# UDC-GAC/pRIblast

Measured on AMD Instinct MI355X. Metric: query RNAs/sec in `ris` step, higher is better.
Workload: dtype f64

## Files before the change

### priblast_amd/csrc/gapped_front.hip

```cpp
#include <algorithm>
#include <cstdlib>

#include "gapped_args.hpp"
#include "search_device.hpp"
#include "search_kernels.hpp"

namespace prb {

#ifdef PRB_GAP_PROFILE
__device__ unsigned long long g_front_prof[32];
#define FP_DECL unsigned long long fp_t0_ = __builtin_amdgcn_s_memtime(), fp_acc_[32] = {}
#define FP_MARK(k)                                              \
  do {                                                          \
    const unsigned long long t_ = __builtin_amdgcn_s_memtime(); \
    fp_acc_[k] += t_ - fp_t0_;                                  \
    fp_t0_ = t_;                                                \
  } while (0)
#define FP_COUNT(k, v) fp_acc_[k] += (unsigned long long)(v)
#define FP_FLUSH()                                                        \
  do {                                                                    \
    if (lane == 0)                                                        \
      for (int i_ = 0; i_ < 32; i_++) atomicAdd(&g_front_prof[i_], fp_acc_[i_]); \
  } while (0)
#else
#define FP_DECL
#define FP_MARK(k)
#define FP_COUNT(k, v)
#define FP_FLUSH()
#endif

namespace {

constexpr int kFD = kFrontMaxDrop;
#ifndef PRB_FRONT_RING
#define PRB_FRONT_RING 24
#endif
constexpr int kFR = PRB_FRONT_RING;
constexpr int kFWaves = 1;
constexpr int kFDirs = 64;
constexpr int kFCells = 192;
#ifndef PRB_FRONT_PAIRS
#define PRB_FRONT_PAIRS 256
#endif
constexpr int kFPairs = PRB_FRONT_PAIRS;

struct FrontTab {
  static constexpr int kBulge = SearchTab::kInt11;
  static constexpr int kTau = kBulge + 31;
  static constexpr int kZero = kTau + 8;
  static constexpr int kCount = kZero + 1;
};
static_assert(SearchTab::kStack == 0 && SearchTab::kInt11 == 255, "stack, internal and mismatch tables lead SearchTab");

struct FrontAcc {
  double eq[kFD][kFDirs], ed[kFD][kFDirs];
};

#ifndef PRB_FRONT_POOL
#define PRB_FRONT_POOL 832
#endif
constexpr int kFPool = PRB_FRONT_POOL;
static_assert(kFPool >= 2 * kFDirs && kFPool <= 1024, "FRec::pool");
static_assert(kFrontMaxDrop <= 16, "FrontLds::wfp: 16 cells per anti-diagonal");
struct FRec {
  static __device__ __forceinline__ uint32_t pack(int i, int j, int pool, int type, int qa, int da) {
    return (uint32_t)i | ((uint32_t)j << 5) | ((uint32_t)pool << 10) | ((uint32_t)type << 20) | ((uint32_t)qa << 23) | ((uint32_t)da << 26);
  }
  static __device__ __forceinline__ int i(uint32_t v) { return v & 31; }
  static __device__ __forceinline__ int j(uint32_t v) { return (v >> 5) & 31; }
  static __device__ __forceinline__ int pool(uint32_t v) { return (v >> 10) & 1023; }
  static __device__ __forceinline__ int type(uint32_t v) { return (v >> 20) & 7; }
  static __device__ __forceinline__ int qa(uint32_t v) { return (v >> 23) & 7; }
  static __device__ __forceinline__ int da(uint32_t v) { return (v >> 26) & 7; }
};

struct FrontLds {
  double hyb[kFPool];
  double te[kFPairs];
  int32_t tab[FrontTab::kCount];
  uint32_t info[kFR][kFDirs];
  uint32_t cells[kFCells];
  uint32_t wfp[2][kFDirs];
  uint8_t improved[kFDirs];
  uint32_t pairs[kFPairs];
};

struct Planes {
  uint32_t lo, hi, valid;
};
__device__ __forceinline__ int plane_base(uint32_t lo, uint32_t hi, uint32_t valid, int t) {
  const uint32_t l = (lo >> t) & 1, h = (hi >> t) & 1, v = (valid >> t) & 1;
  return v ? (int)(((h * 2 + l + 2) & 3) + 1) : 0;
}

__device__ __forceinline__ Planes load_planes(const uint8_t *s, int64_t n, int64_t start, int dir) {
  Planes p{0, 0, 0};
  const int64_t first = dir > 0 ? start : start - 31;
  const uintptr_t addr = reinterpret_cast<uintptr_t>(s) + (uintptr_t)first;
  const int sh = (int)(addr & 3);
  const uint32_t *sw = reinterpret_cast<const uint32_t *>(addr - (uintptr_t)sh);
  uint32_t w[9];
#pragma unroll
  for (int k = 0; k < 9; k++) {
    const int64_t pos_lo = first - sh + 4 * k;
    w[k] = (pos_lo + 3 >= 0 && pos_lo < n) ? sw[k] : 0u;
  }
  uint32_t x[8];
#pragma unroll
  for (int k = 0; k < 8; k++) x[k] = __builtin_amdgcn_alignbyte(w[k + 1], w[k], (uint32_t)sh);
#pragma unroll
  for (int k = 0; k < 8; k++) {
    const uint32_t c = x[k];
    const uint32_t any = (c | (c >> 1) | (c >> 2)) >> 1;
    const uint32_t lo4 = ((c & 0x01010101u) * 0x10204080u) >> 28;
    const uint32_t hi4 = (((c >> 1) & 0x01010101u) * 0x10204080u) >> 28;
    const uint32_t ok4 = ((any & 0x01010101u) * 0x10204080u) >> 28;
    p.lo |= lo4 << (4 * k);
    p.hi |= hi4 << (4 * k);
    p.valid |= ok4 << (4 * k);
  }
  {
    const int64_t lo_t = first < 0 ? -first : 0;
    const int64_t hi_t = first + 31 >= n ? n - 1 - first : 31;
    uint32_t inside = 0;
    if (hi_t >= lo_t) inside = (hi_t >= 31 ? ~0u : ((1u << (hi_t + 1)) - 1u)) & ~((1u << lo_t) - 1u);
    p.valid &= inside;
  }
  if (dir < 0) {
    p.lo = __builtin_bitreverse32(p.lo);
    p.hi = __builtin_bitreverse32(p.hi);
    p.valid = __builtin_bitreverse32(p.valid);
  }
  p.lo &= p.valid;
  p.hi &= p.valid;
  return p;
}

__device__ __forceinline__ void diag_masks(const Planes &q, const Planes &dr, int len, uint32_t &pairs, uint32_t &wob) {
  const int s = 31 - len;
  const uint32_t dl = dr.lo >> s, dh = dr.hi >> s, dv = dr.valid >> s;
  const uint32_t both = q.valid & dv, ldiff = q.lo ^ dl;
  const uint32_t gu = ~(q.hi | dh);
  wob = both & ldiff & gu;
  pairs = both & ldiff & ((q.hi ^ dh) | gu);
}

__device__ __forceinline__ int wave_excl_scan(int v, int lane, int &total) {
  int x = v;
  x += __builtin_amdgcn_update_dpp(0, x, 0x111, 0xF, 0xF, true);
  x += __builtin_amdgcn_update_dpp(0, x, 0x112, 0xF, 0xF, true);
  x += __builtin_amdgcn_update_dpp(0, x, 0x114, 0xF, 0xF, true);
  x += __builtin_amdgcn_update_dpp(0, x, 0x118, 0xF, 0xF, true);
  x += __builtin_amdgcn_update_dpp(0, x, 0x142, 0xA, 0xF, false);
  x += __builtin_amdgcn_update_dpp(0, x, 0x143, 0xC, 0xF, false);
  (void)lane;
  total = __builtin_amdgcn_readlane(x, 63);
  return x - v;
}

__device__ __forceinline__ void wave_lds_sync() {
  __builtin_amdgcn_fence(__ATOMIC_RELEASE, "wavefront");
  __builtin_amdgcn_wave_barrier();
  __builtin_amdgcn_fence(__ATOMIC_ACQUIRE, "wavefront");
}
__device__ __forceinline__ void wave_mem_sync() {
  __builtin_amdgcn_fence(__ATOMIC_RELEASE, "workgroup");
  __builtin_amdgcn_wave_barrier();
  __builtin_amdgcn_fence(__ATOMIC_ACQUIRE, "workgroup");
}

__device__ __forceinline__ double loop_energy_front(const SearchConst &sc, const int32_t *lt, int type, int type2, int u1, int u2, int a,
                                                    int b, int c, int d) {
  using T = SearchTab;
  using F = FrontTab;
  const int tt = type * 8 + type2;
  const int st = T::kStack + type * 7 + type2;
  const bool z1 = u1 == 0, z2 = u2 == 0;
  const int u = z1 ? u2 : u1;
  const bool c11 = u1 == 1 && u2 == 1, c12 = u1 == 1 && u2 == 2, c21 = u1 == 2 && u2 == 1, c22 = u1 == 2 && u2 == 2;
  const bool special = c11 || c12 || c21 || c22;
  int i1 = T::kInternal + u1 + u2;
  int i2 = special ? F::kZero : T::kMismatchI + (type * 5 + a) * 5 + b;
  int i3 = special ? F::kZero : T::kMismatchI + (type2 * 5 + d) * 5 + c;
  if (z1 || z2) {
    const bool stack = z1 && z2;
    i1 = stack ? st : F::kBulge + u;
    i2 = stack ? F::kZero : (u == 1 ? st : F::kTau + type);
    i3 = (stack || u == 1) ? F::kZero : F::kTau + type2;
  }
  int z1v = lt[special ? F::kZero : i1];
  if (special) {
    const int i11 = T::kInt11 + (tt * 5 + a) * 5 + b;
    const int i21a = T::kInt21 + ((tt * 5 + a) * 5 + d) * 5 + b;
    const int i21b = T::kInt21 + (((type2 * 8 + type) * 5 + d) * 5 + a) * 5 + c;
    const int i22 = T::kInt22 + (((tt * 5 + a) * 5 + c) * 5 + d) * 5 + b;
    z1v = sc.tab[c11 ? i11 : c12 ? i21a : c21 ? i21b : i22];
  }
  return div100(sc, z1v + lt[i2] + lt[i3]);
}

template <bool kOneDir>
__global__ __launch_bounds__(64 * kFWaves) void k_gapped_front(GapArgs a, FrontAcc *acc_blocks) {
  __shared__ FrontLds lds[kFWaves];
  const int lane = threadIdx.x & 63;
  FrontLds &S = lds[threadIdx.x >> 6];
  FrontAcc &A = acc_blocks[(int64_t)blockIdx.x * kFWaves + (threadIdx.x >> 6)];
  const SearchConst &sc = a.sc;
  for (int t = lane; t < FrontTab::kCount; t += 64)
    S.tab[t] = t < SearchTab::kInt11    ? sc.tab[t]
               : t < FrontTab::kTau     ? sc.tab[SearchTab::kBulge + (t - FrontTab::kBulge)]
               : t < FrontTab::kZero    ? sc.tab[SearchTab::kTau + (t - FrontTab::kTau)]
                                        : 0;
  const int flag = kOneDir ? 1 : lane & 1;
  const bool f0 = flag == 0;
  const int drop = a.o.drop_w_gap, min_helix = a.o.min_helix, delta = a.o.delta;
  const int64_t nwaves = (int64_t)gridDim.x * kFWaves;
  constexpr int kTileHits = kOneDir ? kFDirs : kFDirs / 2;
  const int64_t ntiles = (a.n + kTileHits - 1) / kTileHits;
  const bool isdir = lane < kFDirs;
  const int me = isdir ? lane : 0;
  int64_t tile = (int64_t)blockIdx.x * kFWaves + (threadIdx.x >> 6);
  FP_DECL;
  while (tile < ntiles) {
    FP_MARK(0);
    FP_COUNT(16, 1);
    unsigned long long nt = 0;
    if (lane == 0) nt = atomicAdd(a.next_work, 1ull);
    const int64_t w = tile * kTileHits + (kOneDir ? lane : lane >> 1);
    const bool live = isdir && w < a.n;
    int64_t x = 0, qo = 0, dbase = 0;
    int query = 0, id = 0, qn = 1, q_sp = 0, db_sp = 0, q_len = 0, db_len = 0, id_start = 0;
    double e_tot = 0, e_acc = 0;
    bool resumed = false;
    int tier0 = 0, nleft0 = 0;
    if (live) {
      x = a.subset ? (int64_t)a.subset[w] : w;
      query = a.in.query[x];
      qo = a.qb.off[query];
      qn = a.qb.len[query] + 1;
      id = a.in.db_id[x];
      dbase = (int64_t)a.pg.start_pos[id] - id;
      q_sp = a.in.q_sp[x];
      db_sp = a.in.db_sp[x];
      q_len = a.in.q_len[x];
      db_len = a.in.db_len[x];
      id_start = a.in.db_id_start[x];
      e_tot = a.in.e_tot[x];
      e_acc = a.in.e_acc[x];
      const uint8_t mark = a.tier_out[x];
      if (is_resumed(mark)) {
        resumed = true;
        tier0 = mark & kMarkTier;
        nleft0 = a.bp_count[x] & 0xFFFF;
        q_sp = a.out.q_sp[x];
        db_sp = a.out.db_sp[x];
        q_len = a.out.q_len[x];
        db_len = a.out.db_len[x];
        id_start = a.out.db_id_start[x];
        e_tot = a.out.e_tot[x];
        e_acc = a.out.e_acc[x];
      }
    }
    const uint8_t *qs = a.qb.enc + qo;
    const int q_start = f0 ? q_sp : q_sp + US(q_len) - 1;
    const int64_t db_start = f0 ? (int64_t)db_sp : (int64_t)db_sp + US(db_len) - 1;
    const int id_end = id_start + US(db_len) - 1;
    bool dead = !live || (resumed && f0);
    if (kOneDir && !resumed) dead = true;
    FP_MARK(1);

    Planes q{0, 0, 0}, dr{0, 0, 0};
    int tq0 = 1, td0 = 1;
    int type0 = 0, q1 = 0, d1 = 0;
    if (live) {
      q = load_planes(qs, qn, q_start, f0 ? -1 : 1);
      const Planes dd = load_planes(a.pg.seqs, a.pg.nchars, db_start, f0 ? -1 : 1);
      tq0 = (q.valid >> 1) == 0x7FFFFFFFu ? 32 : __builtin_ctz(~(q.valid >> 1)) + 1;
      td0 = (dd.valid >> 1) == 0x7FFFFFFFu ? 32 : __builtin_ctz(~(dd.valid >> 1)) + 1;
      const int q0 = plane_base(q.lo, q.hi, q.valid, 0), d0 = plane_base(dd.lo, dd.hi, dd.valid, 0);
      q1 = plane_base(q.lo, q.hi, q.valid, 1);
      d1 = plane_base(dd.lo, dd.hi, dd.valid, 1);
      type0 = bp_type(sc, q0, d0);
      if (f0) type0 = rtype_of(type0);
      dr.lo = __builtin_bitreverse32(dd.lo);
      dr.hi = __builtin_bitreverse32(dd.hi);
      dr.valid = __builtin_bitreverse32(dd.valid);
    }
    FP_MARK(2);
    const int open_until = tq0 > td0 ? tq0 : td0;
    const int lend = drop < open_until ? drop : open_until;

    {
      const float *a3 = f0 ? a.qb.acc + qo : a.pg.acc + dbase, *c3 = f0 ? a.qb.cond + qo : a.pg.cond + dbase;
      const float *c1 = f0 ? a.pg.cond + dbase + id_end : a.qb.cond + qo + q_start;
      const int p0 = f0 ? q_start : id_start;
      const int t3 = f0 ? tq0 : td0, t1 = f0 ? td0 : tq0;
      double s3 = 0, s1 = 0;
      float ta[kFD + 1], tz[kFD], tw[kFD];
      ta[0] = (live && 1 < t3 && 1 <= lend) ? a3[p0] : 0.0f;
#pragma unroll
      for (int len = 1; len <= kFD; len++) {
        const bool v3 = live && len < t3 && len <= lend, v1 = live && len < t1 && len <= lend;
        ta[len] = v3 ? a3[p0 - len] : 0.0f;
        tz[len - 1] = v3 ? c3[p0 - len + delta] : 0.0f;
        tw[len - 1] = v1 ? c1[len] : 0.0f;
      }
#pragma unroll
      for (int len = 1; len <= kFD; len++) {
        const float xx = ta[len], yy = ta[len - 1], zz = tz[len - 1], ww = tw[len - 1];
        s3 = len == 1 ? (double)(xx - yy + zz) : s3 + xx - yy + zz;
        s1 = len == 1 ? (double)ww : s1 + ww;
        if (isdir) {
          A.eq[len - 1][lane] = f0 ? s3 : s1;
          A.ed[len - 1][lane] = f0 ? s1 : s3;
        }
      }
    }
    if (isdir) {
      S.hyb[lane] = e_tot;
      S.info[0][lane] = FRec::pack(0, 0, lane, type0, q1, d1);
      S.improved[lane] = 0;
    }
    int nrec = 1;
    int pool_used = kFDirs;
    uint32_t F2 = type0 != 0 ? 1u : 0u, W2 = wobble(type0) ? 1u : 0u, F1 = 0, W1 = 0;
    wave_mem_sync();
    FP_MARK(3);

    for (int LA = 2; LA <= kFD; LA += 2) {
      if (__ballot(!dead && LA <= lend) == 0) break;
      FP_COUNT(17, 1);
      uint32_t fA = 0, fB = 0;
#pragma unroll
      for (int h = 0; h < 2; h++) {
        const int L = LA + h;
        uint32_t p0, wb0, ahead = ~0u;
        diag_masks(q, dr, L, p0, wb0);
        for (int xx = 1; xx <= min_helix - 1; xx++) {
          uint32_t px, wbx;
          Planes qx{q.lo >> xx, q.hi >> xx, q.valid >> xx};
          diag_masks(qx, dr, L + xx, px, wbx);
          ahead &= px;
          if (xx == 1) ahead &= ~(wb0 & wbx);
        }
        const uint32_t Fp = h == 0 ? F2 : F1, Wp = h == 0 ? W2 : W1;
        const uint32_t need = ~(Fp << 1) | (wb0 & (Wp << 1));
        const int i_first = L - td0 + 1 > 1 ? L - td0 + 1 : 1;
        const int i_hi = (L < tq0 ? L : tq0) - 1;
        const uint32_t range = i_hi >= i_first ? (((i_hi >= 31 ? ~0u : ((1u << (i_hi + 1)) - 1))) & ~((1u << i_first) - 1)) : 0u;
        const uint32_t f = (!dead && L <= lend) ? (p0 & (ahead | ~need) & range) : 0u;
        if (h == 0) fA = f;
        else fB = f;
      }
      int cnt = __popc(fA) + __popc(fB);
      FP_MARK(4);
      if (nrec + cnt > kFR) {
        FP_COUNT(21, __popcll(__ballot(nrec + cnt > kFR)));
        dead = true;
        fA = fB = 0;
        cnt = 0;
      }
      int total;
      int base = wave_excl_scan(cnt, lane, total);
      if (total > kFCells || pool_used + total > kFPool) {
        if (base + cnt > kFCells || pool_used + base + cnt > kFPool) {
          dead = true;
          fA = fB = 0;
          cnt = 0;
        }
        base = wave_excl_scan(cnt, lane, total);
      }
      {
        int r = 0;
        for (uint32_t m = fA; m; m &= m - 1, r++) S.cells[base + r] = (uint32_t)lane | ((uint32_t)__builtin_ctz(m) << 8) | ((uint32_t)(nrec + r) << 16);
        for (uint32_t m = fB; m; m &= m - 1, r++)
          S.cells[base + r] = (uint32_t)lane | ((uint32_t)__builtin_ctz(m) << 8) | (1u << 13) | ((uint32_t)(nrec + r) << 16);
      }
      if (isdir) {
        S.wfp[0][lane] = 0;
        S.wfp[1][lane] = 0;
      }
      wave_lds_sync();
      FP_MARK(5);
      FP_COUNT(19, total);

      for (int c0 = 0; c0 < total;) {
        FP_COUNT(18, 1);
        const bool has = c0 + lane < total;
        const uint32_t cell = has ? S.cells[c0 + lane] : 0u;
        const int dl = cell & 63, ci = (cell >> 8) & 31, isB = (cell >> 13) & 1, rec = (int)(cell >> 16);
        const int cj = LA + isB - ci;
        const bool cf0 = !kOneDir && (dl & 1) == 0;
        const uint32_t cq_lo = __shfl(q.lo, dl), cq_hi = __shfl(q.hi, dl), cq_v = __shfl(q.valid, dl);
        const uint32_t cd_lo = __shfl(dr.lo, dl), cd_hi = __shfl(dr.hi, dl), cd_v = __shfl(dr.valid, dl);
        const int nrecb = __shfl(nrec, dl);
        const int qc = plane_base(cq_lo, cq_hi, cq_v, ci), nq = plane_base(cq_lo, cq_hi, cq_v, ci > 0 ? ci - 1 : 0),
                  fq = plane_base(cq_lo, cq_hi, cq_v, ci + 1);
        const int sh = 31 - cj - 1;
        const uint32_t dlo = cd_lo >> (sh & 31), dhi = cd_hi >> (sh & 31), dvv = cd_v >> (sh & 31);
        const int fd = plane_base(dlo, dhi, dvv, 0), dc = plane_base(dlo, dhi, dvv, 1), nd = plane_base(dlo, dhi, dvv, 2);
        int ctype = bp_type(sc, qc, dc);
        if (!cf0) ctype = rtype_of(ctype);
        uint32_t qmask = 0;
        double eqc = 0, edc = 0;
        if (has) {
          eqc = A.eq[ci - 1][dl];
          edc = A.ed[cj - 1][dl];
        }
        const int nscan = has ? nrecb : 0;
        for (int k = 0; __ballot(k < nscan) != 0; k += 2) {
          const uint32_t v0 = S.info[k][dl], v1 = S.info[k + 1 < kFR ? k + 1 : k][dl];
          if (k < nscan && FRec::i(v0) < ci && FRec::j(v0) < cj) qmask |= 1u << k;
          if (k + 1 < nscan && FRec::i(v1) < ci && FRec::j(v1) < cj) qmask |= 2u << k;
        }
        const uint32_t cdw = (uint32_t)ci | ((uint32_t)cj << 5) | ((uint32_t)ctype << 10) | ((uint32_t)nq << 13) | ((uint32_t)nd << 16) |
                             ((uint32_t)dl << 19);
        const int pool = pool_used + c0 + lane;
        if (has) S.info[rec][dl] = FRec::pack(ci, cj, pool, rtype_of(ctype), fq, fd);
        FP_MARK(6);
        int npc = __popc(qmask), ptotal;
        int poff = wave_excl_scan(npc, lane, ptotal);
        const unsigned long long fits = __ballot(has && poff + npc <= kFPairs);
        const int ncr = fits == ~0ull ? 64 : __builtin_ctzll(~fits);
        const bool mine = lane < ncr;
        if (ncr < 64) ptotal = __shfl(poff, ncr);
        if (mine) {
          int r = 0;
          for (uint32_t m = qmask; m; m &= m - 1, r++) S.pairs[poff + r] = cdw | ((uint32_t)__builtin_ctz(m) << 25);
        }
        wave_lds_sync();
        FP_MARK(7);
        FP_COUNT(20, ptotal);
        for (int p0 = 0; p0 < ptotal; p0 += 64) {
          const int p = p0 + lane;
          if (p < ptotal) {
            const uint32_t cdv = S.pairs[p];
            const int k = cdv >> 25;
            const int pci = cdv & 31, pcj = (cdv >> 5) & 31, pct = (cdv >> 10) & 7, pnq = (cdv >> 13) & 7, pnd = (cdv >> 16) & 7,
                      pdl = (cdv >> 19) & 63;
            const bool pf0 = !kOneDir && (pdl & 1) == 0;
            const uint32_t v = S.info[k][pdl];
            const double hk = S.hyb[FRec::pool(v)];
            const int ri = FRec::i(v), rj = FRec::j(v), rq = FRec::qa(v), rd = FRec::da(v), rt = FRec::type(v);
            double te = loop_energy_front(sc, S.tab, pf0 ? pct : rt, pf0 ? rt : pct, pci - ri - 1, pcj - rj - 1, pf0 ? pnq : rq,
                                          pf0 ? pnd : rd, pf0 ? rq : pnq, pf0 ? rd : pnd);
            te += hk;
            S.te[p] = te;
          }
        }
        wave_lds_sync();
        FP_MARK(8);
        if (mine) {
          double bte = 1000000.0;
          int bk = 0;
          int r = 0;
          for (uint32_t m = qmask; m; m &= m - 1, r++) {
            const double te = S.te[poff + r];
            if (te < bte) {
              bte = te;
              bk = __builtin_ctz(m);
            }
          }
          const int ptype = FRec::type(S.info[bk][dl]);
          S.hyb[pool] = bte;
          if (ptype != 0) atomicOr(&S.wfp[isB][dl], (wobble(ptype) ? 0x10001u : 1u) << (ci - 1));
          const double ie = eqc + edc + bte;
          const double min_e = S.hyb[dl];
          if (ie < min_e) S.improved[dl] = 1;
        }
        wave_lds_sync();
        FP_MARK(9);
        c0 += ncr;
      }
      nrec += cnt;
      pool_used += total;
      {
        const uint32_t m0 = S.wfp[0][me], m1 = S.wfp[1][me];
        F2 = (m0 & 0xFFFFu) << 1;
        W2 = (m0 >> 16) << 1;
        F1 = (m1 & 0xFFFFu) << 1;
        W1 = (m1 >> 16) << 1;
      }
      FP_COUNT(22, __popcll(__ballot(!dead && S.improved[me] != 0)));
      if (S.improved[me]) dead = true;
      FP_MARK(10);
    }

    FP_COUNT(23, pool_used > 640);
    FP_COUNT(24, pool_used > 704);
    FP_COUNT(25, pool_used > 768);
    FP_COUNT(26, pool_used);
    FP_MARK(11);
    bool ok = live && (!dead || (resumed && f0));
    bool ok_other;
    double dng = 0, dng_other = 0;
    if constexpr (kOneDir) {
      ok_other = ok;
      ok = live && resumed;
      if (live) {
        dng = dangle_energy_gapped(sc, q_sp, (int64_t)db_sp, 0, qs, qn, a.pg.seqs, a.pg.nchars);
        dng_other = dangle_energy_gapped(sc, q_sp + US(q_len) - 1, (int64_t)db_sp + US(db_len) - 1, 1, qs, qn, a.pg.seqs, a.pg.nchars);
      }
    } else {
      ok_other = __shfl_xor(ok ? 1 : 0, 1) != 0;
      if (live) {
        const int qp = f0 ? q_sp : q_sp + US(q_len) - 1;
        const int64_t dp = f0 ? (int64_t)db_sp : (int64_t)db_sp + US(db_len) - 1;
        dng = dangle_energy_gapped(sc, qp, dp, flag, qs, qn, a.pg.seqs, a.pg.nchars);
      }
      dng_other = __shfl_xor(dng, 1);
    }
    if (live && (kOneDir || f0)) {
      if (ok && ok_other) {
        const double d0 = dng, d1 = dng_other;
        double e = e_tot, hy = e_tot - e_acc;
        e += d0;
        e += d1;
        hy += d0;
        hy += d1;
        a.overflow[w] = 0;
        a.tier_out[x] = (uint8_t)(resumed ? tier0 : a.tier_id);
        a.bp_count[x] = nleft0;
        a.out.q_sp[x] = q_sp;
        a.out.db_sp[x] = db_sp;
        a.out.q_len[x] = q_len;
        a.out.db_len[x] = db_len;
        a.out.db_id[x] = id;
        a.out.db_id_start[x] = id_start;
        a.out.query[x] = query;
        a.out.e_acc[x] = e_acc;
        a.out.e_hyb[x] = hy;
        a.out.e_tot[x] = e;
      } else {
        a.overflow[w] = 1;
        if (resumed) {
          a.tier_out[x] = (uint8_t)(kResumeMark | tier0);
        } else if (ok) {
          a.out.q_sp[x] = q_sp;
          a.out.db_sp[x] = db_sp;
          a.out.q_len[x] = q_len;
          a.out.db_len[x] = db_len;
          a.out.db_id_start[x] = id_start;
          a.out.e_acc[x] = e_acc;
          a.out.e_hyb[x] = e_tot - e_acc;
          a.out.e_tot[x] = e_tot;
          a.bp_count[x] = 0;
          a.tier_out[x] = kResumeMark;
        }
      }
    }
    wave_mem_sync();
    tile = nwaves + (int64_t)__shfl(nt, 0);
    FP_MARK(12);
  }
  FP_FLUSH();
}

}

#ifdef PRB_GAP_PROFILE
extern "C" int prb_debug_front_profile(unsigned long long *out, int reset) {
  if (hipDeviceSynchronize() != hipSuccess) return -1;
  if (hipMemcpyFromSymbol(out, HIP_SYMBOL(g_front_prof), sizeof(unsigned long long) * 32) != hipSuccess) return -1;
  if (reset) {
    unsigned long long z[32] = {};
    if (hipMemcpyToSymbol(HIP_SYMBOL(g_front_prof), z, sizeof(z)) != hipSuccess) return -1;
  }
  return 0;
}
#endif

bool gapped_front_supported(const SearchConst &sc, const ExtOpts &o) {
  uint32_t pm = 0, wm = 0;
  auto set = [&](uint32_t &m, int q, int d) { m |= 1u << (q * 5 + d); };
  set(pm, 1, 4), set(pm, 4, 1), set(pm, 2, 3), set(pm, 3, 2), set(pm, 3, 4), set(pm, 4, 3);
  set(wm, 3, 4), set(wm, 4, 3);
  return sc.pair_mask == pm && sc.wobble_mask == wm && o.min_helix >= 1 && o.min_helix <= 7 && o.drop_w_gap >= 1 &&
         o.drop_w_gap <= kFD;
}

static int front_blocks_per_cu() {
  const size_t granule = 2048, lds = (sizeof(FrontLds) * kFWaves + granule - 1) / granule * granule;
  return std::max<int>(1, std::min<int>(12, (int)((160 * 1024) / lds)));
}
size_t gapped_front_scratch_bytes() { return (size_t)256 * front_blocks_per_cu() * kFWaves * sizeof(FrontAcc); }

hipError_t launch_gapped_front(const HitSoA &in, HitSoA out, int64_t n, const uint32_t *subset, const QBatchDev &qb, const PageDev &pg,
                               const SearchConst &sc, ExtOpts o, int tier_id, uint8_t *overflow, uint8_t *tier_out, int32_t *bp_count,
                               unsigned long long *next_work, void *scratch, hipStream_t s, bool second_only) {
  if (n <= 0) return hipSuccess;
  GapArgs a{in,      out,     n,       subset,    qb, pg, sc, o, overflow, tier_out, tier_id, nullptr, bp_count,
            nullptr, nullptr, nullptr, next_work, GapResume{nullptr, nullptr, nullptr, 0}, GapResume{nullptr, nullptr, nullptr, 0}};
  if (hipError_t e = hipMemsetAsync(next_work, 0, sizeof(unsigned long long), s); e != hipSuccess) return e;
  const int per_tile = second_only ? kFDirs : kFDirs / 2;
  const int64_t tiles = (n + per_tile - 1) / per_tile, want_blocks = (tiles + kFWaves - 1) / kFWaves;
  const dim3 grid((unsigned)std::min<int64_t>(want_blocks, 256 * front_blocks_per_cu())), blk(64 * kFWaves);
  if (second_only) hipLaunchKernelGGL(k_gapped_front<true>, grid, blk, 0, s, a, static_cast<FrontAcc *>(scratch));
  else hipLaunchKernelGGL(k_gapped_front<false>, grid, blk, 0, s, a, static_cast<FrontAcc *>(scratch));
  return hipGetLastError();
}

}
```

Before: 7.490.

## Shrink front-kernel LDS and registers to fit more wavefronts per CU

Packs the per-wave LDS more tightly: the pairs and te arrays share storage through a union, cells become 16-bit, the improved flags become a bitmask, the pool shrinks, and the score table is shared across two waves per workgroup. Per-hit metadata is reloaded from global memory after the front loop instead of being held in registers, and the accumulator prefix loop is processed in groups of eight to lower register pressure. It also sets waves_per_eu and fixes the count at ten waves per CU. The intent is higher occupancy to hide latency, at the cost of a block-level barrier, redundant global reloads, and more pool overflows from the smaller pool.

```diff
diff --git a/priblast_amd/csrc/gapped_front.hip b/priblast_amd/csrc/gapped_front.hip
--- a/priblast_amd/csrc/gapped_front.hip
+++ b/priblast_amd/csrc/gapped_front.hip
@@ -36,7 +36,7 @@
 #define PRB_FRONT_RING 24
 #endif
 constexpr int kFR = PRB_FRONT_RING;
-constexpr int kFWaves = 1;
+constexpr int kFWaves = 2;
 constexpr int kFDirs = 64;
 constexpr int kFCells = 192;
 #ifndef PRB_FRONT_PAIRS
@@ -57,7 +57,7 @@
 };
 
 #ifndef PRB_FRONT_POOL
-#define PRB_FRONT_POOL 832
+#define PRB_FRONT_POOL 768
 #endif
 constexpr int kFPool = PRB_FRONT_POOL;
 static_assert(kFPool >= 2 * kFDirs && kFPool <= 1024, "FRec::pool");
@@ -74,16 +74,29 @@
   static __device__ __forceinline__ int da(uint32_t v) { return (v >> 26) & 7; }
 };
 
+union FPair {
+  uint32_t pair;
+  double te;
+};
 struct FrontLds {
   double hyb[kFPool];
-  double te[kFPairs];
+  FPair pr[kFPairs];
+  uint32_t info[kFR][kFDirs];
+  uint32_t wfp[2][kFDirs];
+  uint32_t improved[kFDirs / 32];
+  uint16_t cells[kFCells];
+};
+static_assert(kFDirs == 64 && kFR <= 32, "FrontLds::cells: 6 + 4 + 1 + 5 bits");
+struct FrontBlockLds {
+  FrontLds w[kFWaves];
   int32_t tab[FrontTab::kCount];
-  uint32_t info[kFR][kFDirs];
-  uint32_t cells[kFCells];
-  uint32_t wfp[2][kFDirs];
-  uint8_t improved[kFDirs];
-  uint32_t pairs[kFPairs];
-};
+};
+constexpr int kFrontWavesPerCu = 10;
+constexpr size_t kFrontLdsPerCu = 160 * 1024, kFrontLdsGranule = 1280;
+static_assert(kFrontWavesPerCu % kFWaves == 0, "whole workgroups");
+static_assert((sizeof(FrontBlockLds) + kFrontLdsGranule - 1) / kFrontLdsGranule * kFrontLdsGranule * (kFrontWavesPerCu / kFWaves) <= kFrontLdsPerCu,
+              "FrontBlockLds: kFrontWavesPerCu wavefronts no longer fit a compute unit's LDS");
+static_assert(sizeof(FrontBlockLds) <= 16384 * kFWaves, "FrontBlockLds: at most 16 KB per wavefront");
 
 struct Planes {
   uint32_t lo, hi, valid;
@@ -199,18 +212,57 @@
   return div100(sc, z1v + lt[i2] + lt[i3]);
 }
 
+struct FrontHit {
+  int64_t x = 0, qo = 0, dbase = 0;
+  int query = 0, id = 0, qn = 1, q_sp = 0, db_sp = 0, q_len = 0, db_len = 0, id_start = 0;
+  double e_tot = 0, e_acc = 0;
+  bool resumed = false;
+  int tier0 = 0, nleft0 = 0;
+};
+__device__ __forceinline__ FrontHit front_load_hit(const GapArgs &a, int64_t w, bool live) {
+  FrontHit h;
+  if (live) {
+    const int64_t x = a.subset ? (int64_t)a.subset[w] : w;
+    h.x = x;
+    h.query = a.in.query[x];
+    h.qo = a.qb.off[h.query];
+    h.qn = a.qb.len[h.query] + 1;
+    h.id = a.in.db_id[x];
+    h.dbase = (int64_t)a.pg.start_pos[h.id] - h.id;
+    const uint8_t mark = a.tier_out[x];
+    h.resumed = is_resumed(mark);
+    const HitSoA &f = h.resumed ? a.out : a.in;
+    h.q_sp = f.q_sp[x];
+    h.db_sp = f.db_sp[x];
+    h.q_len = f.q_len[x];
+    h.db_len = f.db_len[x];
+    h.id_start = f.db_id_start[x];
+    h.e_tot = f.e_tot[x];
+    h.e_acc = f.e_acc[x];
+    if (h.resumed) {
+      h.tier0 = mark & kMarkTier;
+      h.nleft0 = a.bp_count[x] & 0xFFFF;
+    }
+  }
+  return h;
+}
+
+constexpr int kFAccGroup = 8;
+static_assert(kFD % kFAccGroup == 0, "whole groups");
+
 template <bool kOneDir>
-__global__ __launch_bounds__(64 * kFWaves) void k_gapped_front(GapArgs a, FrontAcc *acc_blocks) {
-  __shared__ FrontLds lds[kFWaves];
+__global__ __launch_bounds__(64 * kFWaves) __attribute__((amdgpu_waves_per_eu(3))) void k_gapped_front(GapArgs a, FrontAcc *acc_blocks) {
+  __shared__ FrontBlockLds lds;
   const int lane = threadIdx.x & 63;
-  FrontLds &S = lds[threadIdx.x >> 6];
+  FrontLds &S = lds.w[threadIdx.x >> 6];
   FrontAcc &A = acc_blocks[(int64_t)blockIdx.x * kFWaves + (threadIdx.x >> 6)];
   const SearchConst &sc = a.sc;
-  for (int t = lane; t < FrontTab::kCount; t += 64)
-    S.tab[t] = t < SearchTab::kInt11    ? sc.tab[t]
-               : t < FrontTab::kTau     ? sc.tab[SearchTab::kBulge + (t - FrontTab::kBulge)]
-               : t < FrontTab::kZero    ? sc.tab[SearchTab::kTau + (t - FrontTab::kTau)]
-                                        : 0;
+  for (int t = threadIdx.x; t < FrontTab::kCount; t += 64 * kFWaves)
+    lds.tab[t] = t < SearchTab::kInt11    ? sc.tab[t]
+                 : t < FrontTab::kTau     ? sc.tab[SearchTab::kBulge + (t - FrontTab::kBulge)]
+                 : t < FrontTab::kZero    ? sc.tab[SearchTab::kTau + (t - FrontTab::kTau)]
+                                          : 0;
+  __syncthreads();
   const int flag = kOneDir ? 1 : lane & 1;
   const bool f0 = flag == 0;
   const int drop = a.o.drop_w_gap, min_helix = a.o.min_helix, delta = a.o.delta;
@@ -226,104 +278,81 @@
     FP_COUNT(16, 1);
     unsigned long long nt = 0;
     if (lane == 0) nt = atomicAdd(a.next_work, 1ull);
-    const int64_t w = tile * kTileHits + (kOneDir ? lane : lane >> 1);
-    const bool live = isdir && w < a.n;
-    int64_t x = 0, qo = 0, dbase = 0;
-    int query = 0, id = 0, qn = 1, q_sp = 0, db_sp = 0, q_len = 0, db_len = 0, id_start = 0;
-    double e_tot = 0, e_acc = 0;
-    bool resumed = false;
-    int tier0 = 0, nleft0 = 0;
-    if (live) {
-      x = a.subset ? (int64_t)a.subset[w] : w;
-      query = a.in.query[x];
-      qo = a.qb.off[query];
-      qn = a.qb.len[query] + 1;
-      id = a.in.db_id[x];
-      dbase = (int64_t)a.pg.start_pos[id] - id;
-      q_sp = a.in.q_sp[x];
-      db_sp = a.in.db_sp[x];
-      q_len = a.in.q_len[x];
-      db_len = a.in.db_len[x];
-      id_start = a.in.db_id_start[x];
-      e_tot = a.in.e_tot[x];
-      e_acc = a.in.e_acc[x];
-      const uint8_t mark = a.tier_out[x];
-      if (is_resumed(mark)) {
-        resumed = true;
-        tier0 = mark & kMarkTier;
-        nleft0 = a.bp_count[x] & 0xFFFF;
-        q_sp = a.out.q_sp[x];
-        db_sp = a.out.db_sp[x];
-        q_len = a.out.q_len[x];
-        db_len = a.out.db_len[x];
-        id_start = a.out.db_id_start[x];
-        e_tot = a.out.e_tot[x];
-        e_acc = a.out.e_acc[x];
-      }
-    }
-    const uint8_t *qs = a.qb.enc + qo;
-    const int q_start = f0 ? q_sp : q_sp + US(q_len) - 1;
-    const int64_t db_start = f0 ? (int64_t)db_sp : (int64_t)db_sp + US(db_len) - 1;
-    const int id_end = id_start + US(db_len) - 1;
-    bool dead = !live || (resumed && f0);
-    if (kOneDir && !resumed) dead = true;
-    FP_MARK(1);
-
+    bool dead;
     Planes q{0, 0, 0}, dr{0, 0, 0};
-    int tq0 = 1, td0 = 1;
-    int type0 = 0, q1 = 0, d1 = 0;
-    if (live) {
-      q = load_planes(qs, qn, q_start, f0 ? -1 : 1);
-      const Planes dd = load_planes(a.pg.seqs, a.pg.nchars, db_start, f0 ? -1 : 1);
-      tq0 = (q.valid >> 1) == 0x7FFFFFFFu ? 32 : __builtin_ctz(~(q.valid >> 1)) + 1;
-      td0 = (dd.valid >> 1) == 0x7FFFFFFFu ? 32 : __builtin_ctz(~(dd.valid >> 1)) + 1;
-      const int q0 = plane_base(q.lo, q.hi, q.valid, 0), d0 = plane_base(dd.lo, dd.hi, dd.valid, 0);
-      q1 = plane_base(q.lo, q.hi, q.valid, 1);
-      d1 = plane_base(dd.lo, dd.hi, dd.valid, 1);
-      type0 = bp_type(sc, q0, d0);
-      if (f0) type0 = rtype_of(type0);
-      dr.lo = __builtin_bitreverse32(dd.lo);
-      dr.hi = __builtin_bitreverse32(dd.hi);
-      dr.valid = __builtin_bitreverse32(dd.valid);
-    }
-    FP_MARK(2);
-    const int open_until = tq0 > td0 ? tq0 : td0;
-    const int lend = drop < open_until ? drop : open_until;
-
+    int tq0 = 1, td0 = 1, lend;
+    uint32_t F2, W2, F1 = 0, W1 = 0;
     {
-      const float *a3 = f0 ? a.qb.acc + qo : a.pg.acc + dbase, *c3 = f0 ? a.qb.cond + qo : a.pg.cond + dbase;
-      const float *c1 = f0 ? a.pg.cond + dbase + id_end : a.qb.cond + qo + q_start;
-      const int p0 = f0 ? q_start : id_start;
-      const int t3 = f0 ? tq0 : td0, t1 = f0 ? td0 : tq0;
+      const int64_t w = tile * kTileHits + (kOneDir ? lane : lane >> 1);
+      const bool live = isdir && w < a.n;
+      const FrontHit h = front_load_hit(a, w, live);
+      const uint8_t *qs = a.qb.enc + h.qo;
+      const int q_start = f0 ? h.q_sp : h.q_sp + US(h.q_len) - 1;
+      const int64_t db_start = f0 ? (int64_t)h.db_sp : (int64_t)h.db_sp + US(h.db_len) - 1;
+      const int id_end = h.id_start + US(h.db_len) - 1;
+      dead = !live || (h.resumed && f0);
+      if (kOneDir && !h.resumed) dead = true;
+      FP_MARK(1);
+
+      int type0 = 0, q1 = 0, d1 = 0;
+      if (live) {
+        q = load_planes(qs, h.qn, q_start, f0 ? -1 : 1);
+        const Planes dd = load_planes(a.pg.seqs, a.pg.nchars, db_start, f0 ? -1 : 1);
+        tq0 = (q.valid >> 1) == 0x7FFFFFFFu ? 32 : __builtin_ctz(~(q.valid >> 1)) + 1;
+        td0 = (dd.valid >> 1) == 0x7FFFFFFFu ? 32 : __builtin_ctz(~(dd.valid >> 1)) + 1;
+        const int q0 = plane_base(q.lo, q.hi, q.valid, 0), d0 = plane_base(dd.lo, dd.hi, dd.valid, 0);
+        q1 = plane_base(q.lo, q.hi, q.valid, 1);
+        d1 = plane_base(dd.lo, dd.hi, dd.valid, 1);
+        type0 = bp_type(sc, q0, d0);
+        if (f0) type0 = rtype_of(type0);
+        dr.lo = __builtin_bitreverse32(dd.lo);
+        dr.hi = __builtin_bitreverse32(dd.hi);
+        dr.valid = __builtin_bitreverse32(dd.valid);
+      }
+      FP_MARK(2);
+      const int open_until = tq0 > td0 ? tq0 : td0;
+      lend = drop < open_until ? drop : open_until;
+      if (isdir) {
+        S.hyb[lane] = h.e_tot;
+        S.info[0][lane] = FRec::pack(0, 0, lane, type0, q1, d1);
+      }
+      if (lane < kFDirs / 32) S.improved[lane] = 0;
+      F2 = type0 != 0 ? 1u : 0u;
+      W2 = wobble(type0) ? 1u : 0u;
+
+      const float *a3 = (f0 ? a.qb.acc + h.qo : a.pg.acc + h.dbase) + (f0 ? q_start : h.id_start);
+      const float *c3 = (f0 ? a.qb.cond + h.qo : a.pg.cond + h.dbase) + (f0 ? q_start : h.id_start) + delta;
+      const float *c1 = f0 ? a.pg.cond + h.dbase + id_end : a.qb.cond + h.qo + q_start;
+      const int n3 = live ? min(f0 ? tq0 : td0, lend + 1) : 0, n1 = live ? min(f0 ? td0 : tq0, lend + 1) : 0;
       double s3 = 0, s1 = 0;
-      float ta[kFD + 1], tz[kFD], tw[kFD];
-      ta[0] = (live && 1 < t3 && 1 <= lend) ? a3[p0] : 0.0f;
+      float yy = 1 < n3 ? a3[0] : 0.0f;
+      double *oq = &A.eq[0][lane], *od = &A.ed[0][lane];
+#pragma unroll 1
+      for (int l0 = 1; l0 <= kFD; l0 += kFAccGroup) {
+        float ta[kFAccGroup], tz[kFAccGroup], tw[kFAccGroup];
 #pragma unroll
-      for (int len = 1; len <= kFD; len++) {
-        const bool v3 = live && len < t3 && len <= lend, v1 = live && len < t1 && len <= lend;
-        ta[len] = v3 ? a3[p0 - len] : 0.0f;
-        tz[len - 1] = v3 ? c3[p0 - len + delta] : 0.0f;
-        tw[len - 1] = v1 ? c1[len] : 0.0f;
-      }
+        for (int g = 0; g < kFAccGroup; g++) {
+          const int len = l0 + g;
+          ta[g] = len < n3 ? a3[-len] : 0.0f;
+          tz[g] = len < n3 ? c3[-len] : 0.0f;
+          tw[g] = len < n1 ? c1[len] : 0.0f;
+        }
 #pragma unroll
-      for (int len = 1; len <= kFD; len++) {
-        const float xx = ta[len], yy = ta[len - 1], zz = tz[len - 1], ww = tw[len - 1];
-        s3 = len == 1 ? (double)(xx - yy + zz) : s3 + xx - yy + zz;
-        s1 = len == 1 ? (double)ww : s1 + ww;
-        if (isdir) {
-          A.eq[len - 1][lane] = f0 ? s3 : s1;
-          A.ed[len - 1][lane] = f0 ? s1 : s3;
-        }
-      }
-    }
-    if (isdir) {
-      S.hyb[lane] = e_tot;
-      S.info[0][lane] = FRec::pack(0, 0, lane, type0, q1, d1);
-      S.improved[lane] = 0;
+        for (int g = 0; g < kFAccGroup; g++) {
+          const float xx = ta[g], zz = tz[g], ww = tw[g];
+          const bool first = l0 + g == 1;
+          s3 = first ? (double)(xx - yy + zz) : s3 + xx - yy + zz;
+          s1 = first ? (double)ww : s1 + ww;
+          yy = xx;
+          if (isdir) {
+            oq[(l0 + g - 1) * kFDirs] = f0 ? s3 : s1;
+            od[(l0 + g - 1) * kFDirs] = f0 ? s1 : s3;
+          }
+        }
+      }
     }
     int nrec = 1;
     int pool_used = kFDirs;
-    uint32_t F2 = type0 != 0 ? 1u : 0u, W2 = wobble(type0) ? 1u : 0u, F1 = 0, W1 = 0;
     wave_mem_sync();
     FP_MARK(3);
 
@@ -363,6 +392,8 @@
       int total;
       int base = wave_excl_scan(cnt, lane, total);
       if (total > kFCells || pool_used + total > kFPool) {
+        FP_COUNT(27, total > kFCells);
+        FP_COUNT(28, pool_used + total > kFPool);
         if (base + cnt > kFCells || pool_used + base + cnt > kFPool) {
           dead = true;
           fA = fB = 0;
@@ -372,9 +403,10 @@
       }
       {
         int r = 0;
-        for (uint32_t m = fA; m; m &= m - 1, r++) S.cells[base + r] = (uint32_t)lane | ((uint32_t)__builtin_ctz(m) << 8) | ((uint32_t)(nrec + r) << 16);
+        const uint32_t c = (uint32_t)lane | ((uint32_t)nrec << 11);
+        for (uint32_t m = fA; m; m &= m - 1, r++) S.cells[base + r] = (uint16_t)(c + ((uint32_t)(__builtin_ctz(m) - 1) << 6) + ((uint32_t)r << 11));
         for (uint32_t m = fB; m; m &= m - 1, r++)
-          S.cells[base + r] = (uint32_t)lane | ((uint32_t)__builtin_ctz(m) << 8) | (1u << 13) | ((uint32_t)(nrec + r) << 16);
+          S.cells[base + r] = (uint16_t)(c + ((uint32_t)(__builtin_ctz(m) - 1) << 6) + (1u << 10) + ((uint32_t)r << 11));
       }
       if (isdir) {
         S.wfp[0][lane] = 0;
@@ -388,7 +420,7 @@
         FP_COUNT(18, 1);
         const bool has = c0 + lane < total;
         const uint32_t cell = has ? S.cells[c0 + lane] : 0u;
-        const int dl = cell & 63, ci = (cell >> 8) & 31, isB = (cell >> 13) & 1, rec = (int)(cell >> 16);
+        const int dl = cell & 63, ci = ((cell >> 6) & 15) + 1, isB = (cell >> 10) & 1, rec = (int)(cell >> 11);
         const int cj = LA + isB - ci;
         const bool cf0 = !kOneDir && (dl & 1) == 0;
         const uint32_t cq_lo = __shfl(q.lo, dl), cq_hi = __shfl(q.hi, dl), cq_v = __shfl(q.valid, dl);
@@ -426,7 +458,7 @@
         if (ncr < 64) ptotal = __shfl(poff, ncr);
         if (mine) {
           int r = 0;
-          for (uint32_t m = qmask; m; m &= m - 1, r++) S.pairs[poff + r] = cdw | ((uint32_t)__builtin_ctz(m) << 25);
+          for (uint32_t m = qmask; m; m &= m - 1, r++) S.pr[poff + r].pair = cdw | ((uint32_t)__builtin_ctz(m) << 25);
         }
         wave_lds_sync();
         FP_MARK(7);
@@ -434,7 +466,7 @@
         for (int p0 = 0; p0 < ptotal; p0 += 64) {
           const int p = p0 + lane;
           if (p < ptotal) {
-            const uint32_t cdv = S.pairs[p];
+            const uint32_t cdv = S.pr[p].pair;
             const int k = cdv >> 25;
             const int pci = cdv & 31, pcj = (cdv >> 5) & 31, pct = (cdv >> 10) & 7, pnq = (cdv >> 13) & 7, pnd = (cdv >> 16) & 7,
                       pdl = (cdv >> 19) & 63;
@@ -442,10 +474,10 @@
             const uint32_t v = S.info[k][pdl];
             const double hk = S.hyb[FRec::pool(v)];
             const int ri = FRec::i(v), rj = FRec::j(v), rq = FRec::qa(v), rd = FRec::da(v), rt = FRec::type(v);
-            double te = loop_energy_front(sc, S.tab, pf0 ? pct : rt, pf0 ? rt : pct, pci - ri - 1, pcj - rj - 1, pf0 ? pnq : rq,
+            double te = loop_energy_front(sc, lds.tab, pf0 ? pct : rt, pf0 ? rt : pct, pci - ri - 1, pcj - rj - 1, pf0 ? pnq : rq,
                                           pf0 ? pnd : rd, pf0 ? rq : pnq, pf0 ? rd : pnd);
             te += hk;
-            S.te[p] = te;
+            S.pr[p].te = te;
           }
         }
         wave_lds_sync();
@@ -455,7 +487,7 @@
           int bk = 0;
           int r = 0;
           for (uint32_t m = qmask; m; m &= m - 1, r++) {
-            const double te = S.te[poff + r];
+            const double te = S.pr[poff + r].te;
             if (te < bte) {
               bte = te;
               bk = __builtin_ctz(m);
@@ -466,7 +498,7 @@
           if (ptype != 0) atomicOr(&S.wfp[isB][dl], (wobble(ptype) ? 0x10001u : 1u) << (ci - 1));
           const double ie = eqc + edc + bte;
           const double min_e = S.hyb[dl];
-          if (ie < min_e) S.improved[dl] = 1;
+          if (ie < min_e) atomicOr(&S.improved[dl >> 5], 1u << (dl & 31));
         }
         wave_lds_sync();
         FP_MARK(9);
@@ -481,71 +513,79 @@
         F1 = (m1 & 0xFFFFu) << 1;
         W1 = (m1 >> 16) << 1;
       }
-      FP_COUNT(22, __popcll(__ballot(!dead && S.improved[me] != 0)));
-      if (S.improved[me]) dead = true;
+      const bool improved = ((S.improved[me >> 5] >> (me & 31)) & 1u) != 0;
+      FP_COUNT(22, __popcll(__ballot(!dead && improved)));
+      if (improved) dead = true;
       FP_MARK(10);
     }
 
-    FP_COUNT(23, pool_used > 640);
-    FP_COUNT(24, pool_used > 704);
-    FP_COUNT(25, pool_used > 768);
+    FP_COUNT(23, pool_used > 576);
+    FP_COUNT(24, pool_used > 640);
+    FP_COUNT(25, pool_used > 704);
     FP_COUNT(26, pool_used);
     FP_MARK(11);
-    bool ok = live && (!dead || (resumed && f0));
-    bool ok_other;
-    double dng = 0, dng_other = 0;
-    if constexpr (kOneDir) {
-      ok_other = ok;
-      ok = live && resumed;
-      if (live) {
-        dng = dangle_energy_gapped(sc, q_sp, (int64_t)db_sp, 0, qs, qn, a.pg.seqs, a.pg.nchars);
-        dng_other = dangle_energy_gapped(sc, q_sp + US(q_len) - 1, (int64_t)db_sp + US(db_len) - 1, 1, qs, qn, a.pg.seqs, a.pg.nchars);
-      }
-    } else {
-      ok_other = __shfl_xor(ok ? 1 : 0, 1) != 0;
-      if (live) {
-        const int qp = f0 ? q_sp : q_sp + US(q_len) - 1;
-        const int64_t dp = f0 ? (int64_t)db_sp : (int64_t)db_sp + US(db_len) - 1;
-        dng = dangle_energy_gapped(sc, qp, dp, flag, qs, qn, a.pg.seqs, a.pg.nchars);
-      }
-      dng_other = __shfl_xor(dng, 1);
-    }
-    if (live && (kOneDir || f0)) {
-      if (ok && ok_other) {
-        const double d0 = dng, d1 = dng_other;
-        double e = e_tot, hy = e_tot - e_acc;
-        e += d0;
-        e += d1;
-        hy += d0;
-        hy += d1;
-        a.overflow[w] = 0;
-        a.tier_out[x] = (uint8_t)(resumed ? tier0 : a.tier_id);
-        a.bp_count[x] = nleft0;
-        a.out.q_sp[x] = q_sp;
-        a.out.db_sp[x] = db_sp;
-        a.out.q_len[x] = q_len;
-        a.out.db_len[x] = db_len;
-        a.out.db_id[x] = id;
-        a.out.db_id_start[x] = id_start;
-        a.out.query[x] = query;
-        a.out.e_acc[x] = e_acc;
-        a.out.e_hyb[x] = hy;
-        a.out.e_tot[x] = e;
+    {
+      const int64_t w = tile * kTileHits + (kOneDir ? lane : lane >> 1);
+      const bool live = isdir && w < a.n;
+      const FrontHit h = front_load_hit(a, w, live);
+      const uint8_t *qs = a.qb.enc + h.qo;
+      const int64_t x = h.x;
+      bool ok = live && (!dead || (h.resumed && f0));
+      bool ok_other;
+      double dng = 0, dng_other = 0;
+      if constexpr (kOneDir) {
+        ok_other = ok;
+        ok = live && h.resumed;
+        if (live) {
+          dng = dangle_energy_gapped(sc, h.q_sp, (int64_t)h.db_sp, 0, qs, h.qn, a.pg.seqs, a.pg.nchars);
+          dng_other = dangle_energy_gapped(sc, h.q_sp + US(h.q_len) - 1, (int64_t)h.db_sp + US(h.db_len) - 1, 1, qs, h.qn, a.pg.seqs, a.pg.nchars);
+        }
       } else {
-        a.overflow[w] = 1;
-        if (resumed) {
-          a.tier_out[x] = (uint8_t)(kResumeMark | tier0);
-        } else if (ok) {
-          a.out.q_sp[x] = q_sp;
-          a.out.db_sp[x] = db_sp;
-          a.out.q_len[x] = q_len;
-          a.out.db_len[x] = db_len;
-          a.out.db_id_start[x] = id_start;
-          a.out.e_acc[x] = e_acc;
-          a.out.e_hyb[x] = e_tot - e_acc;
-          a.out.e_tot[x] = e_tot;
-          a.bp_count[x] = 0;
-          a.tier_out[x] = kResumeMark;
+        ok_other = __shfl_xor(ok ? 1 : 0, 1) != 0;
+        if (live) {
+          const int qp = f0 ? h.q_sp : h.q_sp + US(h.q_len) - 1;
+          const int64_t dp = f0 ? (int64_t)h.db_sp : (int64_t)h.db_sp + US(h.db_len) - 1;
+          dng = dangle_energy_gapped(sc, qp, dp, flag, qs, h.qn, a.pg.seqs, a.pg.nchars);
+        }
+        dng_other = __shfl_xor(dng, 1);
+      }
+      if (live && (kOneDir || f0)) {
+        if (ok && ok_other) {
+          const double d0 = dng, d1 = dng_other;
+          double e = h.e_tot, hy = h.e_tot - h.e_acc;
+          e += d0;
+          e += d1;
+          hy += d0;
+          hy += d1;
+          a.overflow[w] = 0;
+          a.tier_out[x] = (uint8_t)(h.resumed ? h.tier0 : a.tier_id);
+          a.bp_count[x] = h.nleft0;
+          a.out.q_sp[x] = h.q_sp;
+          a.out.db_sp[x] = h.db_sp;
+          a.out.q_len[x] = h.q_len;
+          a.out.db_len[x] = h.db_len;
+          a.out.db_id[x] = h.id;
+          a.out.db_id_start[x] = h.id_start;
+          a.out.query[x] = h.query;
+          a.out.e_acc[x] = h.e_acc;
+          a.out.e_hyb[x] = hy;
+          a.out.e_tot[x] = e;
+        } else {
+          a.overflow[w] = 1;
+          if (h.resumed) {
+            a.tier_out[x] = (uint8_t)(kResumeMark | h.tier0);
+          } else if (ok) {
+            a.out.q_sp[x] = h.q_sp;
+            a.out.db_sp[x] = h.db_sp;
+            a.out.q_len[x] = h.q_len;
+            a.out.db_len[x] = h.db_len;
+            a.out.db_id_start[x] = h.id_start;
+            a.out.e_acc[x] = h.e_acc;
+            a.out.e_hyb[x] = h.e_tot - h.e_acc;
+            a.out.e_tot[x] = h.e_tot;
+            a.bp_count[x] = 0;
+            a.tier_out[x] = kResumeMark;
+          }
         }
       }
     }
@@ -579,10 +619,7 @@
          o.drop_w_gap <= kFD;
 }
 
-static int front_blocks_per_cu() {
-  const size_t granule = 2048, lds = (sizeof(FrontLds) * kFWaves + granule - 1) / granule * granule;
-  return std::max<int>(1, std::min<int>(12, (int)((160 * 1024) / lds)));
-}
+static int front_blocks_per_cu() { return kFrontWavesPerCu / kFWaves; }
 size_t gapped_front_scratch_bytes() { return (size_t)256 * front_blocks_per_cu() * kFWaves * sizeof(FrontAcc); }
 
 hipError_t launch_gapped_front(const HitSoA &in, HitSoA out, int64_t n, const uint32_t *subset, const QBatchDev &qb, const PageDev &pg,
```

New measurement: 7.638 (median of 6 runs). +2.0%, better.
